# vb000/LookOnceToHear

Measured on AMD Instinct MI355X. Metric: frames_per_sec (5 s 16 kHz binaural clips, 625 STFT frames each, offline forward), higher is better.
Workload: dtype f32 via f16x3 split (3x fp16 MFMA per product, fp32 accumulate; ~22-bit operands, un-normalised rows scaled by a power of two before the split: any finite fp32 range); 1 GPU; BASELINE configs[2]: 32 x 5 s 16 kHz binaural clips per GPU, offline forward (configs/tsh.json separator, random-init weights); batch_per_gpu=32, global_batch=32, parallelism=utterance-dp1, gemm_mode=f16x3, tune=, batches_in_flight=1

## Files before the change

include/lookonce_hip.h:

```cpp
#ifndef LOOKONCE_HIP_H
#define LOOKONCE_HIP_H

#ifdef __cplusplus
extern "C" {
#endif

typedef void* lh_stream_t;

enum {
    LH_OK = 0,
    LH_ERR_ARG = 1,
    LH_ERR_UNSUPPORTED = 2,
    LH_ERR_LAUNCH = 3,
    LH_ERR_RANGE = 4
};

int lh_range_status(unsigned* range_flag, lh_stream_t stream);
int lh_range_flag_copy(unsigned* range_flag, void* host_pinned, lh_stream_t stream);
int lh_range_flag_clear(unsigned* range_flag, lh_stream_t stream);
int lh_selftest_fp16_subnormal(lh_stream_t stream);

enum { LH_GEMM_F32 = 0, LH_GEMM_F16X3 = 1 };

int lh_abi_version(void);
// ... 54 lines not shown
int lh_ring_advance_rows(int* pos, const int* write_pos, int modulo, int n_rows, lh_stream_t stream);

int lh_proj_ln_res(const float* merged, const void* w_pk, const float* bias, const float* slope,
                   const float* ln_w, const float* ln_b, const float* y2, const float* gain, float* out, int B,
                   int T, lh_stream_t stream);
int lh_proj_ln_res_fan(const float* merged, const void* w_pk, const float* bias, const float* slope, const float* ln_w,
                       const float* ln_b, const float* y2, const float* gain, float* out, int B, int T, int K,
                       lh_stream_t stream);
int lh_proj_ln_res_fan_win(const float* merged, const void* w_pk, const float* bias, const float* slope, const float* ln_w,
                           const float* ln_b, const float* y2, const float* gain, float* out, int B, int T, int t0, int Tc,
                           int K, lh_stream_t stream);

int lh_deconv_istft(const float* y, const float* deconv_buf_in, float* deconv_buf_out, const float* istft_buf_in,
                    float* istft_buf_out, const void* wdec_pk, const float* bdec, const void* wfb_dec,
                    float* wave_out, unsigned* range_flag, int keep_nonfinite, int B, int T, lh_stream_t stream);

int lh_intra_block_win(const float* x, const void* w_pk, const float* b_sum, const void* wlin_pk, const float* blin,
                       float* out, int B, int T, int t0, int Tc, lh_stream_t stream);
int lh_inter_block_win(const float* x, const void* w_pk, const float* b_sum, const void* wlin_pk, const float* blin,
                       const float* h0, const float* c0, float* hN, float* cN, float* out, int B, int T, int t0, int Tc,
                       int carry, lh_stream_t stream);
int lh_ln_lstm_intra_win(const float* x, const float* ln_w, const float* ln_b, const void* w_pk, const float* b_sum, float* h_out,
                         int B, int T, int t0, int Tc, lh_stream_t stream);
int lh_linear_res_win(const float* h, const void* w_pk, const float* bias, const float* res, float* out, int B, int T, int t0,
                      int Tc, int K, lh_stream_t stream);
int lh_inter_matvec_win(const float* x, const void* wih_pk, const float* b_sum, const float* whh, const void* wlin_pk,
                        const float* blin, const float* h0, const float* c0, float* hN, float* cN, float* out, int B, int T,
                        int t0, int Tc, int carry, lh_stream_t stream);
int lh_qkv_proj_ln_win(const float* y, const void* w_pk, const float* bias, const float* slopes, const float* lnq_w,
                       const float* lnq_b, const float* lnk_w, const float* lnk_b, const float* lnv_w,
// ... 153 lines not shown
```

lookoncetohear_amd/_cabi.py:

```python
from __future__ import annotations

import ctypes
import os
from ctypes import c_double, c_int, c_ulonglong, c_void_p

_PKG = os.path.dirname(os.path.abspath(__file__))
HIP_LIB_PATH = os.path.join(_PKG, "_lookonce_hip.so")
ABI_VERSION = 25

_P, _I = c_void_p, c_int
SIGNATURES = {
    "lh_abi_version": [],
    "lh_check_config": [_I] * 10,
    "lh_stft_conv_in": [_P] * 7 + [_I] * 3 + [_P],
    "lh_embed_proj_ln": [_P] * 7 + [_I, _P],
    "lh_set_tuning": [_I, _I],
    "lh_ln_lstm_intra": [_P] * 6 + [_I, _I, _P],
    "lh_ln_lstm_inter": [_P] * 10 + [_I, _I, _I, _P],
    "lh_intra_stream": [_P] * 5 + [_I, _P],
    "lh_inter_matvec": [_P] * 11 + [_I, _I, _P],
    "lh_intra_block": [_P] * 6 + [_I, _P],
    "lh_inter_block": [_P] * 10 + [_I, _I, _P],
    "lh_linear_res": [_P] * 5 + [_I, _I, _P],
    "lh_qkv_proj_ln": [_P] * 14 + [_I, _I, _P],
# ... 26 lines not shown
    "lh_resample": [_P, _P, _P] + [_I] * 6 + [_P],
    "lh_session_resample_in": [_P, _I, _P, _I, _P, _P, _I, _I, _P, _I, _I, _I, _P],
    "lh_session_resample_out": [_P, _P, _P, _P, _I, _I, _P, _I, _I, _I, _P],
    "lh_proj_ln_res": [_P] * 9 + [_I, _I, _P],
    "lh_deconv_istft": [_P] * 10 + [_I, _I, _I, _P],
    "lh_intra_block_win": [_P] * 6 + [_I, _I, _I, _I, _P],
    "lh_inter_block_win": [_P] * 10 + [_I, _I, _I, _I, _I, _P],
    "lh_ln_lstm_intra_win": [_P] * 6 + [_I, _I, _I, _I, _P],
    "lh_linear_res_win": [_P] * 5 + [_I, _I, _I, _I, _I, _P],
    "lh_inter_matvec_win": [_P] * 11 + [_I, _I, _I, _I, _I, _P],
    "lh_qkv_proj_ln_win": [_P] * 14 + [_I, _I, _I, _I, _P],
    "lh_local_attn_win": [_P] * 4 + [_I, _I, _I, _I, _P],
    "lh_proj_ln_res_win": [_P] * 9 + [_I, _I, _I, _I, _P],
    "lh_proj_ln_res_fan": [_P] * 9 + [_I, _I, _I, _P],
    "lh_proj_ln_res_fan_win": [_P] * 9 + [_I, _I, _I, _I, _I, _P],
    "lh_emb_frontend": [_P] * 10 + [_I, _I, _I, _P],
    "lh_emb_axis_fused": [_P] * 8 + [_I, _I, _I, _I, _I, _P],
    "lh_emb_axis_mv": [_P] * 9 + [_I, _I, _I, _I, _P],
    "lh_emb_attn_block": [_P] * 24 + [_I, _I, _P],
    "lh_emb_head": [_P] * 7 + [_I, _I, _P],
    "lh_render_binaural": [_P] * 8 + [_I, _I, _I, _I, _P],
    "lh_path_nearest": [_P] * 4 + [_I] * 5 + [_P],
    "lh_render_moving": [_P] * 10 + [_I] * 8 + [_P],
    "lh_metric_sums": [_P] * 8 + [_I, _I, _I, _P],
    "lh_binaural_cues": [_P] * 5 + [_I, _I, _I, _I, c_double, _P],
    "lh_range_status": [_P, _P],
    "lh_range_flag_copy": [_P, _P, _P],
    "lh_range_flag_clear": [_P, _P],
    "lh_selftest_fp16_subnormal": [_P],
    "lh_comm_unique_id": [_P],
# ... 119 lines not shown
```

lookoncetohear_amd/csrc/lh_backend.hip:

```cpp
#include "lh_split.h"

namespace lh {

constexpr int BE_NT = 512;
constexpr int BE_TT = 15;
constexpr int BE_NJ = BE_TT + 1;
constexpr int BE_NP = 36;
constexpr int BE_PP = 40;
constexpr int BE_SK = 7;
constexpr int BE_SA = BE_SK * 4 * BE_NJ * 8;
constexpr int BE_FP = NFFT + 4;
constexpr int BE_NLD = (NF * 16 + BE_NT - 1) / BE_NT;
#if !defined(BE_RING_N)
#define BE_RING_N 2
#endif
constexpr int BE_RING = BE_RING_N;
#if defined(LH_PROBE_TRACE)
__device__ unsigned long long lh_be_trace_buf[32];
#if defined(LH_PROBE_TRACE_T1)
#define BE_STAMP(k) do { if (blockIdx.x == 0 && tid == 0) lh_be_trace_buf[k] = __builtin_amdgcn_s_memtime(); } while (0)
#else
#define BE_STAMP(k) do { if (blockIdx.x == 3 && tid == 0 && tk == k0_ + 2) lh_be_trace_buf[k] = __builtin_amdgcn_s_memtime(); } while (0)
#endif
#else
// ... 336 lines not shown
            wave_out[((long)b * NSRC + s) * L + (long)(t0 + jt) * HOP + n] = (nf && !keep_nonfinite) ? 0.f : v;
            bad |= nf;
        }
        if (bad && range_flag) __hip_atomic_store(range_flag, 1u, __ATOMIC_RELAXED, __HIP_MEMORY_SCOPE_SYSTEM);
        __syncthreads();
        for (int i = tid; i < 2 * (FR_RP - NF) * 16; i += BE_NT) {
            const int img = i / ((FR_RP - NF) * 16), e = i % ((FR_RP - NF) * 16);
            *reinterpret_cast<f16x4*>(&ahi[img * FR_A + a_index<FR_RP>(NF + (e >> 4), (e & 15) * 4)]) = f16x4{0, 0, 0, 0};
        }
        BE_STAMP(10);
        }
        if (++tk == k1) run += gridDim.x;
    }
}

static int g_runs_per_b = 0;
int backend_set_runs(int v) {
    if (v < 0) return LH_ERR_ARG;
    g_runs_per_b = v;
    return LH_OK;
}

}

#if defined(LH_PROBE_TRACE)
extern "C" int lh_probe_be_trace_read(unsigned long long* host_dst) {
    return hipMemcpyFromSymbol(host_dst, HIP_SYMBOL(lh::lh_be_trace_buf), sizeof(lh::lh_be_trace_buf)) == hipSuccess ? 0 : 1;
}
#endif

// ... 4 lines not shown
    using namespace lh;
    if (!y || !deconv_buf_in || !deconv_buf_out || !istft_buf_in || !istft_buf_out || !wdec_pk || !bdec || !wfb_dec ||
        !wave_out || B <= 0 || T <= 0)
        return LH_ERR_ARG;
    if (deconv_buf_in == deconv_buf_out || istft_buf_in == istft_buf_out) return LH_ERR_ARG;
    const int tiles_per_b = (T + BE_TT - 1) / BE_TT;
    int runs_per_b = g_runs_per_b ? g_runs_per_b : 256 / B;
    runs_per_b = runs_per_b < 1 ? 1 : (runs_per_b > tiles_per_b ? tiles_per_b : runs_per_b);
    const int n_runs = B * runs_per_b;
    hipLaunchKernelGGL(k_deconv_istft, dim3(n_runs < 256 ? n_runs : 256), dim3(BE_NT), 0, (hipStream_t)stream, y,
                       deconv_buf_in, deconv_buf_out, istft_buf_in, istft_buf_out, (const _Float16*)wdec_pk, bdec,
                       (const _Float16*)wfb_dec, wave_out, range_flag, keep_nonfinite, B, T, runs_per_b);
    return check_launch();
}

namespace lh {
__global__ void k_range_fetch(unsigned* flag) { flag[1] = atomicExch(&flag[0], 0u); }
}
static int range_fetch(unsigned* flag, lh_stream_t stream) {
    if (!flag) return LH_ERR_ARG;
    hipLaunchKernelGGL(lh::k_range_fetch, dim3(1), dim3(1), 0, (hipStream_t)stream, flag);
    return lh::check_launch();
}
extern "C" int lh_range_flag_copy(unsigned* flag, void* host_pinned, lh_stream_t stream) {
    if (!host_pinned) return LH_ERR_ARG;
    const int rc = range_fetch(flag, stream);
    if (rc != LH_OK) return rc;
    return hipMemcpyAsync(host_pinned, flag + 1, sizeof(unsigned), hipMemcpyDeviceToHost, (hipStream_t)stream) == hipSuccess
               ? LH_OK : LH_ERR_LAUNCH;
}
// ... 40 lines not shown
```

lookoncetohear_amd/csrc/lh_frontend.hip:

```cpp
#include "lh_split.h"

namespace lh {

constexpr int FE_NTH = 512;
constexpr int FE_TT = 14;
constexpr int FE_NJ = 16;
constexpr int FE_AP = NFFT + 8;
constexpr int FE_SP = 68;
constexpr int FE_NT = (NK + 15) / 16;
constexpr int FE_KS = NFFT / 32;
constexpr int FE_OP = C + 4;

__global__ void __launch_bounds__(FE_NTH, 1) k_stft_conv_in(const float* __restrict__ x, const float* __restrict__ cbuf_in,
                                                            float* __restrict__ cbuf_out, const _Float16* __restrict__ wfb_pk,
                                                            const _Float16* __restrict__ wc_pk, const float* __restrict__ bc,
                                                            float* __restrict__ z, int B, int T, int n_samples) {
    __shared__ __attribute__((aligned(16))) _Float16 ahi[NMIC * FE_NJ * FE_AP];
    __shared__ __attribute__((aligned(16))) _Float16 alo[NMIC * FE_NJ * FE_AP];
    __shared__ __attribute__((aligned(16))) _Float16 sth[(NF + 2) * FE_SP];
    __shared__ __attribute__((aligned(16))) _Float16 stl[(NF + 2) * FE_SP];
    __shared__ __attribute__((aligned(16))) float outs[2][NF * FE_OP];
    __shared__ float tmax[FE_NTH / 64];
    const int tid = threadIdx.x, lane = tid & 63, wave = wave_id(tid), g4 = lane >> 4, l15 = lane & 15;

// ... 262 lines not shown
}

extern "C" int lh_embed_proj_ln_rows(const float* embed, const float* w, const float* bias, const float* ln_w,
                                     const float* ln_b, float* scratch, float* gain, const lh_snap_item_t* items, int n_items,
                                     int S, lh_stream_t stream) {
    using namespace lh;
    if (!embed || !w || !bias || !ln_w || !ln_b || !scratch || !gain || scratch == gain || !items || S <= 0 || n_items < 1 ||
        n_items > S)
        return LH_ERR_ARG;
    hipLaunchKernelGGL(k_embed_proj_rows, dim3((C * NF + EP_ROWS - 1) / EP_ROWS, (n_items + EP_NB - 1) / EP_NB), dim3(256), 0,
                       (hipStream_t)stream, embed, w, bias, scratch, items, n_items, S);
    hipLaunchKernelGGL(k_embed_ln_rows, dim3(n_items), dim3(256), 0, (hipStream_t)stream, scratch, ln_w, ln_b, gain, items, S);
    return check_launch();
}

extern "C" int lh_abi_version(void) { return 25; }

extern "C" int lh_check_config(int nfft, int hop, int n_mics, int emb_dim, int n_blocks_unused, int lstm_hidden,
                               int n_heads, int attn_window, int n_srcs, int spk_emb_dim) {
    using namespace lh;
    (void)n_blocks_unused;
    if (nfft != NFFT || hop != HOP || n_mics != NMIC || emb_dim != C || lstm_hidden != H || n_heads != NH ||
        attn_window != WIN || n_srcs != NSRC || spk_emb_dim != SPK)
        return LH_ERR_UNSUPPORTED;
    return LH_OK;
}
```

lookoncetohear_amd/csrc/lh_pointwise.hip:

```cpp
#include "lh_split.h"
#include <type_traits>

namespace lh {

template <int K>
__global__ void __launch_bounds__(256) k_linear_res(const float* __restrict__ h, const _Float16* __restrict__ w_pk,
                                                    const float* __restrict__ bias, const float* __restrict__ res,
                                                    float* __restrict__ out, int rows, int seg, long segstride) {
    auto grow = [&](long r) -> long { return (r / seg) * segstride + r % seg; };
    constexpr int KS = K / 32, RP = 64, CP = C + 4;
    __shared__ __attribute__((aligned(16))) _Float16 ahi[KS * 4 * RP * 8];
    __shared__ __attribute__((aligned(16))) _Float16 alo[KS * 4 * RP * 8];
    __shared__ __attribute__((aligned(16))) float cs[RP * CP];
    const int tid = threadIdx.x, lane = tid & 63, wave = wave_id(tid), g4 = lane >> 4, l15 = lane & 15;

    f16x8 wh[KS], wl[KS];
    load_w<KS>(w_pk, wave, lane, wh, wl);
    const float bz = bias[wave * 16 + l15];

    const int ntiles = (rows + RP - 1) / RP;
    for (int tile = blockIdx.x; tile < ntiles; tile += gridDim.x) {
        const long r0 = (long)tile * RP;
        constexpr int NLD = RP * (K / 4) / 256;
        float4 stg[NLD];
// ... 262 lines not shown
        QKV_STAMP(5);
    }
}
#if defined(LH_PROBE_TRACE)
}
extern "C" int lh_probe_qkv_trace_read(unsigned long long* host_dst) {
    return hipMemcpyFromSymbol(host_dst, HIP_SYMBOL(lh::lh_qkv_trace_buf), sizeof(lh::lh_qkv_trace_buf)) == hipSuccess ? 0 : 1;
}
namespace lh {
#endif

#if defined(LH_DBG_K6)
__device__ unsigned lh_dbg_k6[4];
__device__ float lh_dbg_part[8 * 24 * 256 * 4];
#endif
template <bool FAN>
__global__ void __launch_bounds__(256, 2) k_proj_ln_res(const float* __restrict__ merged, const _Float16* __restrict__ w_pk,
                                                     const float* __restrict__ bias, const float* __restrict__ slope,
                                                     const float* __restrict__ lnw, const float* __restrict__ lnb,
                                                     const float* __restrict__ y2, const float* __restrict__ gain,
                                                     float* __restrict__ out, int T, int nframes, int Tc, int tw0, int nfan) {
    constexpr int YP = C + 4;
    auto gidx = [&](int fr) -> long { return (long)(fr / Tc) * T + tw0 + fr % Tc; };
    __shared__ __attribute__((aligned(16))) _Float16 ahi[FR_A];
    __shared__ __attribute__((aligned(16))) _Float16 alo[FR_A];
    __shared__ __attribute__((aligned(16))) float ys[NF * YP];
    __shared__ float red[4];
    const int tid = threadIdx.x, lane = tid & 63, wave = wave_id(tid), g4 = lane >> 4, l15 = lane & 15;

    f16x8 wh[2], wl[2];
    load_w<2>(w_pk, wave, lane, wh, wl);
    const float bz = bias[wave * 16 + l15];
    const float a = slope[0];
    constexpr int N = NF * C, N4 = N / 4;
    constexpr int NSLOT = (N4 + 255) / 256;
    float4 pw[NSLOT], pb[NSLOT];
#pragma unroll
    for (int k = 0; k < NSLOT; ++k) {
        const int i = min(tid + 256 * k, N4 - 1);
        pw[k] = *reinterpret_cast<const float4*>(&lnw[i * 4]);
        pb[k] = *reinterpret_cast<const float4*>(&lnb[i * 4]);
    }

// ... 80 lines not shown
#pragma unroll
                for (int k = 0; k < NSLOT; ++k)
                    rv[k] = *reinterpret_cast<const float4*>(&gj[(long)min(tid + 256 * k, N4 - 1) * 4]);
#pragma unroll
                for (int k = 0; k < NSLOT; ++k) pin_here(rv[k]);
#pragma unroll
                for (int k = 0; k < NSLOT; ++k) {
                    rv[k].x = v[k].x * rv[k].x; rv[k].y = v[k].y * rv[k].y; rv[k].z = v[k].z * rv[k].z; rv[k].w = v[k].w * rv[k].w;
                }
#pragma unroll
                for (int k = 0; k < NSLOT; ++k) {
                    const int i = tid + 256 * k;
                    if (i < N4) *reinterpret_cast<float4*>(&out[fo + i * 4]) = rv[k];
                }
            }
            continue;
        }
        if (gain) {
#pragma unroll
            for (int k = 0; k < NSLOT; ++k)
                rv[k] = *reinterpret_cast<const float4*>(&gain[(long)b * N + (long)min(tid + 256 * k, N4 - 1) * 4]);
#pragma unroll
            for (int k = 0; k < NSLOT; ++k) {
                v[k].x *= rv[k].x; v[k].y *= rv[k].y; v[k].z *= rv[k].z; v[k].w *= rv[k].w;
            }
        }
#pragma unroll
        for (int k = 0; k < NSLOT; ++k) {
            const int i = tid + 256 * k;
            if (i < N4) *reinterpret_cast<float4*>(&out[fr + i * 4]) = v[k];
// ... 67 lines not shown
        return LH_ERR_ARG;
    hipLaunchKernelGGL(k_qkv_proj_ln<true>, dim3(B < 512 ? B : 512), dim3(256), 0, (hipStream_t)stream, y,
                       (const _Float16*)w_pk, bias, slopes, lnq_w, lnq_b, lnk_w, lnk_b, lnv_w, lnv_b, (_Float16*)q,
                       (_Float16*)kx, (_Float16*)vx, 1, B, write_pos, 1, 0);
    return check_launch();
}

extern "C" int lh_proj_ln_res_win(const float* merged, const void* w_pk, const float* bias, const float* slope,
                                  const float* ln_w, const float* ln_b, const float* y2, const float* gain, float* out,
                                  int B, int T, int t0, int Tc, lh_stream_t stream) {
    using namespace lh;
    if (!merged || !w_pk || !bias || !slope || !ln_w || !ln_b || !y2 || !out || B <= 0 || T <= 0 || t0 < 0 || Tc <= 0 ||
        t0 + Tc > T)
        return LH_ERR_ARG;
    const int nframes = B * Tc;
    hipLaunchKernelGGL(k_proj_ln_res<false>, dim3(nframes < 512 ? nframes : 512), dim3(256), 0, (hipStream_t)stream, merged,
                       (const _Float16*)w_pk, bias, slope, ln_w, ln_b, y2, gain, out, T, nframes, Tc, t0, 1);
    return check_launch();
}

extern "C" int lh_proj_ln_res(const float* merged, const void* w_pk, const float* bias, const float* slope,
                              const float* ln_w, const float* ln_b, const float* y2, const float* gain, float* out,
                              int B, int T, lh_stream_t stream) {
    return lh_proj_ln_res_win(merged, w_pk, bias, slope, ln_w, ln_b, y2, gain, out, B, T, 0, T, stream);
}

extern "C" int lh_proj_ln_res_fan_win(const float* merged, const void* w_pk, const float* bias, const float* slope,
                                      const float* ln_w, const float* ln_b, const float* y2, const float* gain, float* out,
                                      int B, int T, int t0, int Tc, int K, lh_stream_t stream) {
    using namespace lh;
    if (!gain || K < 1) return LH_ERR_ARG;
    if (K == 1) return lh_proj_ln_res_win(merged, w_pk, bias, slope, ln_w, ln_b, y2, gain, out, B, T, t0, Tc, stream);
    if (!merged || !w_pk || !bias || !slope || !ln_w || !ln_b || !y2 || !out || B <= 0 || T <= 0 || t0 < 0 || Tc <= 0 ||
        t0 + Tc > T)
        return LH_ERR_ARG;
    const int nframes = B * Tc;
    hipLaunchKernelGGL(k_proj_ln_res<true>, dim3(nframes < 512 ? nframes : 512), dim3(256), 0, (hipStream_t)stream, merged,
                       (const _Float16*)w_pk, bias, slope, ln_w, ln_b, y2, gain, out, T, nframes, Tc, t0, K);
    return check_launch();
}

extern "C" int lh_proj_ln_res_fan(const float* merged, const void* w_pk, const float* bias, const float* slope,
                                  const float* ln_w, const float* ln_b, const float* y2, const float* gain, float* out,
                                  int B, int T, int K, lh_stream_t stream) {
    return lh_proj_ln_res_fan_win(merged, w_pk, bias, slope, ln_w, ln_b, y2, gain, out, B, T, 0, T, K, stream);
}

#if defined(LH_DBG_K6)
extern "C" int lh_dbg_part_read(float* host) {
    return hipMemcpyFromSymbol(host, HIP_SYMBOL(lh::lh_dbg_part), sizeof(lh::lh_dbg_part)) == hipSuccess ? 0 : 1;
}
extern "C" int lh_dbg_k6_read(unsigned* host4, int reset) {
    if (hipMemcpyFromSymbol(host4, HIP_SYMBOL(lh::lh_dbg_k6), 16) != hipSuccess) return 1;
// ... 5 lines not shown
```

lookoncetohear_amd/net.py:

```python
from __future__ import annotations

import ctypes
import math
import os
from typing import Dict, Optional, Tuple

import numpy as np
import torch
import torch.nn as nn
import torch.nn.functional as F

from . import _cabi
from .weights import KV_PAD_ROWS, QK_PAD, pack_all, unsplit_qk, unsplit_v


def mod_pad(x: torch.Tensor, chunk_size: int, pad: Tuple[int, int]):
    mod = 0
    if x.shape[-1] % chunk_size != 0:
        mod = chunk_size - (x.shape[-1] % chunk_size)
    if mod or pad[0] or pad[1]:
        x = F.pad(x, (pad[0], mod + pad[1]))
    return x, mod


# ... 159 lines not shown
            raise NotImplementedError("only the chunk-causal attention mode of configs/tsh.json is implemented")
        shape = (self.nfft, stft_chunk_size, num_ch, D, H, L, local_atten_len, num_src, embed_dim)
        if shape != (192, 128, 2, 64, 64, 4, 50, 2, 256):
            raise NotImplementedError(
                f"the gfx950 kernels are specialised on the configs/tsh.json shapes; got (nfft, hop, mics, D, H, L, "
                f"window, srcs, embed_dim) = {shape}")
        self.E = math.ceil(512 * 1.0 / self.n_freqs)
        self.V_dim = D // L
        self.tfgridnet = _TFGridNetParams(self.nfft, stft_chunk_size, num_ch, num_src, D, B, H, L, embed_dim)
        self.gemm_mode = os.environ.get("LOOKONCE_GEMM", "f16x3")
        self._check_gemm_mode()
        rc = os.environ.get("LOOKONCE_RANGE_CHECK", "1")
        self.range_check = False if rc == "0" else ("sync" if rc == "sync" else True)
        self._range_flags: Dict[str, torch.Tensor] = {}
        self.fuse_linear = os.environ.get("LOOKONCE_FUSE", "1") != "0"
        self.fuse_intra_min_frames = int(os.environ.get("LOOKONCE_FUSE_INTRA_MIN_FRAMES", "6000"))
        self.inter_matvec_max_seqs = int(os.environ.get("LOOKONCE_MATVEC_MAX_SEQS", "256"))
        self.stream_intra_max_frames = 128
        self.n_cus = 256
        self.time_chunks = int(os.environ.get("LOOKONCE_TIME_CHUNKS", "0"))
        self.time_chunks_small = int(os.environ.get("LOOKONCE_TIME_CHUNKS_SMALL", "0"))
        self.chunk_min_frames = 64
        self._chunk_streams: Dict[str, list] = {}
        self._pack_key = None
        self._packed = None
        self._ws: Dict[tuple, dict] = {}
        self._zeros: Dict[tuple, dict] = {}
        self._blob = None
        self._debug_taps: Optional[dict] = None
        self._prof: Optional[list] = None
# ... 218 lines not shown
                    e1.record()
                    prof.append((name, e0, e1))

            lib_, lib = lib, _Timed

            conv_in = c32(state["conv_buf"]); conv_out = new(conv_in)
            lib.call("lh_stft_conv_in", P(x), P(conv_in), P(conv_out), P(pk["wfb_t"]), P(pk["conv_w"]),
                     P(pk["conv_b"]), P(xa), Bn, T, ns, st)
            lib.call("lh_embed_proj_ln", P(embed), P(pk["emb_w"]), P(pk["emb_b"]), P(pk["emb_ln_w"]),
                     P(pk["emb_ln_b"]), P(ws["gain_raw"]), P(ws["gain"]), Bn, st)
            if taps is not None:
                taps["Z0"], taps["G"] = xa.clone(), ws["gain"].clone()

            mode = 1 if self.gemm_mode == "f16x3" else 0
            K = self._n_time_chunks(Bn, T, mode)
            if K > 1:
                self._blocks_chunked(lib, pk, ws, state, Bn, T, dev, from_zero, want_state, K)
            else:
                self._blocks_whole(lib, pk, ws, state, Bn, T, dev, from_zero, want_state, mode)

            dec_in, ist_in = c32(state["deconv_buf"]), c32(state["istft_buf"])
            dec_out, ist_out = new(dec_in), new(ist_in)
            y = torch.empty(Bn, self.n_srcs, hop * T, device=dev, dtype=torch.float32)
            flag = self._range_flag(dev)
            lib.call("lh_deconv_istft", P(xa), P(dec_in), P(dec_out), P(ist_in), P(ist_out), P(pk["deconv_w"]),
                     P(pk["deconv_b"]), P(pk["wfb_dec"]), P(y), P(flag), 1, Bn, T, st)
            if want_state:
                state["conv_buf"], state["deconv_buf"], state["istft_buf"] = conv_out, dec_out, ist_out
            if self.range_check == "sync" and not self._capturing():
                if self.range_status(dev):
                    raise RuntimeError(self._RANGE_MSG.format("this forward"))
        return y, (state if want_state else None)

    def _separate_many(self, x: torch.Tensor, embeds: torch.Tensor) -> torch.Tensor:
        if self.training and torch.is_grad_enabled():
            raise RuntimeError("lookoncetohear_amd.Net is an inference-only drop-in (forward kernels, no autograd): call "
                               ".eval() and/or run under torch.no_grad(); training stays on the reference model")
        self._check_gemm_mode()
        assert x.shape[1] == self.num_ch, "input must be [B, num_ch, N]"
        Bn, _, n = x.shape
        Kt = embeds.shape[1]
        Bk = Bn * Kt
        embed = embeds.reshape(Bk, -1)
        if self.gemm_mode == "f32all" or self.n_blocks < 2:
            y, _ = self._separate(x.repeat_interleave(Kt, 0), embed, None, False)
            return y.view(Bn, Kt, *y.shape[1:])
        lib = self._lib(x)
# ... 27 lines not shown
                K = self._n_time_chunks(rows, T, mode)
                if K > 1:
                    self._blocks_chunked(lib, pk, w, s, rows, T, dev, True, False, K, blocks, f)
                else:
                    self._blocks_whole(lib, pk, w, s, rows, T, dev, True, False, mode, blocks, f)
            dec_in, ist_in = c32(sk["deconv_buf"]), c32(sk["istft_buf"])
            dec_out, ist_out = new(dec_in), new(ist_in)
            y = torch.empty(Bn, Kt, self.n_srcs, hop * T, device=dev, dtype=torch.float32)
            lib.call("lh_deconv_istft", P(wsk["xa"]), P(dec_in), P(dec_out), P(ist_in), P(ist_out), P(pk["deconv_w"]),
                     P(pk["deconv_b"]), P(pk["wfb_dec"]), P(y), P(self._range_flag(dev)), 1, Bk, T, st)
            if self.range_check == "sync" and not self._capturing():
                if self.range_status(dev):
                    raise RuntimeError(self._RANGE_MSG.format("this forward"))
        return y

    def _blocks_whole(self, lib, pk, ws, state, Bn, T, dev, from_zero, want_state, mode, blocks=None, fan=None):
        F_, nh, H_, hist = self.n_freqs, self.n_head, self.hidden, self.local_atten_len - 1
        P = lambda t: t.data_ptr()
        new = lambda t: torch.empty_like(t, dtype=torch.float32)
        c32 = lambda t: t.contiguous().float()
        xa, xb, xc, hbuf = ws["xa"], ws["xb"], ws["xc"], ws["hbuf"]
        st = self._stream(dev)
        taps = self._debug_taps
        rows = Bn * T * F_
        wkey, bkey = ("_w16", "_b16") if mode else ("_w", "_b")
        for i in (range(self.n_blocks) if blocks is None else blocks):
            bp = pk["blocks"][i]
            bs = state["gridnet_bufs"][f"buf{i}"]
            h0, c0 = c32(bs["h0"]), c32(bs["c0"])
            hN, cN = new(h0), new(c0)
            fuse = mode == 1 and self.fuse_linear
# ... 26 lines not shown
                ws["hist_dirty"] = True
            elif ws["hist_dirty"]:
                ws["kx"][:, :hist].zero_()
                ws["vx"][:, :hist].zero_()
                ws["hist_dirty"] = False
            lib.call("lh_qkv_proj_ln", P(xc), P(bp["qkv_w"]), P(bp["qkv_b"]), P(bp["qkv_slopes"]), P(bp["lnq_w"]),
                     P(bp["lnq_b"]), P(bp["lnk_w"]), P(bp["lnk_b"]), P(bp["lnv_w"]), P(bp["lnv_b"]), P(ws["q"]),
                     P(ws["kx"]), P(ws["vx"]), None, Bn, T, st)
            lib.call("lh_local_attn", P(ws["q"]), P(ws["kx"]), P(ws["vx"]), P(xb), Bn, T, st)
            if taps is not None:
                taps[f"blocks.{i}.attn"] = xb.clone()
            gain = ws["gain"] if (i == 0 and self.n_blocks > 1) else None
            if fan is not None and i == 0:
                lib.call("lh_proj_ln_res_fan", P(xb), P(bp["proj_w"]), P(bp["proj_b"]), P(bp["proj_slope"]),
                         P(bp["proj_ln_w"]), P(bp["proj_ln_b"]), P(xc), P(fan[0]), P(fan[1]), Bn, T, fan[2], st)
            else:
                lib.call("lh_proj_ln_res", P(xb), P(bp["proj_w"]), P(bp["proj_b"]), P(bp["proj_slope"]),
                         P(bp["proj_ln_w"]), P(bp["proj_ln_b"]), P(xc), P(gain) if gain is not None else None, P(xa),
                         Bn, T, st)
            if want_state:
                bs["h0"], bs["c0"] = hN, cN
                bs["K_buf"] = torch.empty(Bn * nh, hist, self.E * F_, device=dev, dtype=torch.float32)
                bs["V_buf"] = torch.empty(Bn * nh, hist, self.V_dim * F_, device=dev, dtype=torch.float32)
                lib.call("lh_ring_unpack", P(ws["kx"]), P(ws["vx"]), P(bs["K_buf"]), P(bs["V_buf"]), Bn, T, st)
            if taps is not None:
                taps[f"blocks.{i}.Y2"] = xc.clone()
                taps[f"blocks.{i}.Q"] = unsplit_qk(ws["q"], self.E * F_)
                taps[f"blocks.{i}.K"] = unsplit_qk(ws["kx"][:, hist:hist + T], self.E * F_)
                taps[f"blocks.{i}.V"] = unsplit_v(ws["vx"][:, hist:hist + T])
                taps[f"blocks.{i}.out"] = xa.clone()
# ... 28 lines not shown
        if Bn * self.n_freqs <= self.inter_matvec_max_seqs:
            align = 64
        cuts = [(k * T) // K for k in range(K + 1)]
        if T // K >= 2 * align or (align == 64 and T // K >= 64):
            cuts = [0] + [int(round(k * T / K / align)) * align for k in range(1, K)] + [T]
        return cuts

    def _lanes(self, dev, K) -> _Lanes:
        pool = self._chunk_streams.setdefault(str(dev), [])
        while len(pool) < K - 1:
            pool.append(torch.cuda.Stream(device=dev))
        if self.chunk_min_frames < self.local_atten_len - 1:
            raise ValueError("chunk_min_frames must cover the attention history (49 frames) on concurrent streams")
        return _Lanes(dev, pool[:K - 1])

    def _blocks_chunked(self, lib, pk, ws, state, Bn, T, dev, from_zero, want_state, K, blocks=None, fan=None):
        blocks = range(self.n_blocks) if blocks is None else blocks
        F_, nh, hist = self.n_freqs, self.n_head, self.local_atten_len - 1
        P = lambda t: t.data_ptr()
        c32 = lambda t: t.contiguous().float()
        xa, xb, xc = ws["xa"], ws["xb"], ws["xc"]
        lanes = self._lanes(dev, K)
        unfused_intra = Bn * T < self.fuse_intra_min_frames
        matvec_inter = Bn * F_ <= self.inter_matvec_max_seqs
        if "kxb" not in ws:
            z16 = lambda *s_: torch.zeros(*s_, device=dev, dtype=torch.float16)
            ws["kxb"] = [ws["kx"]] + [z16(*ws["kx"].shape) for _ in range(self.n_blocks - 1)]
            ws["vxb"] = [ws["vx"]] + [z16(*ws["vx"].shape) for _ in range(self.n_blocks - 1)]
            ws["hist_dirty_b"] = [False] * self.n_blocks
        bounds = self._window_bounds(Bn, T, K)
        hs, cs = {}, {}
# ... 45 lines not shown
                                 t0, Tc, carry, st)
                    if k + 1 < K:
                        ev_r = lanes.signal(k)
                    lib.call("lh_qkv_proj_ln_win", P(xc), P(bp["qkv_w"]), P(bp["qkv_b"]), P(bp["qkv_slopes"]), P(bp["lnq_w"]),
                             P(bp["lnq_b"]), P(bp["lnk_w"]), P(bp["lnk_b"]), P(bp["lnv_w"]), P(bp["lnv_b"]), P(ws["q"]),
                             P(kx), P(vx), None, Bn, T, t0, Tc, st)
                    ev_prev = ev_q
                    if k + 1 < K:
                        ev_q = lanes.signal(k)
                    if k > 0:
                        lanes.wait(k, ev_prev)
                    lib.call("lh_local_attn_win", P(ws["q"]), P(kx), P(vx), P(xb), Bn, T, t0, Tc, st)
                    if fan is not None and i == 0:
                        lib.call("lh_proj_ln_res_fan_win", P(xb), P(bp["proj_w"]), P(bp["proj_b"]), P(bp["proj_slope"]),
                                 P(bp["proj_ln_w"]), P(bp["proj_ln_b"]), P(xc), P(fan[0]), P(fan[1]), Bn, T, t0, Tc, fan[2], st)
                    else:
                        lib.call("lh_proj_ln_res_win", P(xb), P(bp["proj_w"]), P(bp["proj_b"]), P(bp["proj_slope"]),
                                 P(bp["proj_ln_w"]), P(bp["proj_ln_b"]), P(xc), P(gain) if gain is not None else None, P(xa),
                                 Bn, T, t0, Tc, st)
        lanes.join()
        if want_state:
            for i in blocks:
                bs = state["gridnet_bufs"][f"buf{i}"]
                bs["h0"], bs["c0"] = hs[i][K].reshape(1, -1, self.hidden), cs[i][K].reshape(1, -1, self.hidden)
                bs["K_buf"] = torch.empty(Bn * nh, hist, self.E * F_, device=dev, dtype=torch.float32)
                bs["V_buf"] = torch.empty(Bn * nh, hist, self.V_dim * F_, device=dev, dtype=torch.float32)
                lib.call("lh_ring_unpack", P(ws["kxb"][i]), P(ws["vxb"][i]), P(bs["K_buf"]), P(bs["V_buf"]), Bn, T,
                         self._stream(dev))

    def _check_gemm_mode(self):
# ... 1183 lines not shown
```

Baseline: 2.914 million frames/s.

## Fuse deconv tap products into last block's projection and simplify iSTFT kernel

The last block's proj+LN+residual kernel now also computes the 3x3 deconvolution tap products per frequency with MFMA and writes them out with a per-frame max. A new taps_istft kernel then only sums the taps over the time and frequency neighbours, splits the result and runs the synthesis GEMM. This removes the separate deconv GEMM pass over the full-width final features. The cost is an extra intermediate buffer (36 floats per frequency and frame), more shared memory in the projection kernel, and a conservative scaling bound based on the weight norms.

```diff
diff --git a/include/lookonce_hip.h b/include/lookonce_hip.h
--- a/include/lookonce_hip.h
+++ b/include/lookonce_hip.h
@@ -92,6 +92,15 @@
 int lh_deconv_istft(const float* y, const float* deconv_buf_in, float* deconv_buf_out, const float* istft_buf_in,
                     float* istft_buf_out, const void* wdec_pk, const float* bdec, const void* wfb_dec,
                     float* wave_out, unsigned* range_flag, int keep_nonfinite, int B, int T, lh_stream_t stream);
+
+int lh_proj_ln_res_taps(const float* merged, const void* w_pk, const float* bias, const float* slope, const float* ln_w,
+                        const float* ln_b, const float* y2, const void* wdec_pk, float* p_out, float* fmax, int B, int T,
+                        lh_stream_t stream);
+int lh_proj_ln_res_taps_win(const float* merged, const void* w_pk, const float* bias, const float* slope, const float* ln_w,
+                            const float* ln_b, const float* y2, const void* wdec_pk, float* p_out, float* fmax, int B, int T,
+                            int t0, int Tc, lh_stream_t stream);
+int lh_taps_istft(const float* p, const float* fmax, const void* wdec_pk, const float* bdec, const void* wfb_dec,
+                  float* wave_out, unsigned* range_flag, int keep_nonfinite, int B, int T, lh_stream_t stream);
 
 int lh_intra_block_win(const float* x, const void* w_pk, const float* b_sum, const void* wlin_pk, const float* blin,
                        float* out, int B, int T, int t0, int Tc, lh_stream_t stream);
diff --git a/lookoncetohear_amd/_cabi.py b/lookoncetohear_amd/_cabi.py
--- a/lookoncetohear_amd/_cabi.py
+++ b/lookoncetohear_amd/_cabi.py
@@ -6,7 +6,7 @@
 
 _PKG = os.path.dirname(os.path.abspath(__file__))
 HIP_LIB_PATH = os.path.join(_PKG, "_lookonce_hip.so")
-ABI_VERSION = 25
+ABI_VERSION = 26
 
 _P, _I = c_void_p, c_int
 SIGNATURES = {
@@ -64,6 +64,9 @@
     "lh_proj_ln_res_win": [_P] * 9 + [_I, _I, _I, _I, _P],
     "lh_proj_ln_res_fan": [_P] * 9 + [_I, _I, _I, _P],
     "lh_proj_ln_res_fan_win": [_P] * 9 + [_I, _I, _I, _I, _I, _P],
+    "lh_proj_ln_res_taps": [_P] * 10 + [_I, _I, _P],
+    "lh_proj_ln_res_taps_win": [_P] * 10 + [_I, _I, _I, _I, _P],
+    "lh_taps_istft": [_P] * 7 + [_I, _I, _I, _P],
     "lh_emb_frontend": [_P] * 10 + [_I, _I, _I, _P],
     "lh_emb_axis_fused": [_P] * 8 + [_I, _I, _I, _I, _I, _P],
     "lh_emb_axis_mv": [_P] * 9 + [_I, _I, _I, _I, _P],
diff --git a/lookoncetohear_amd/csrc/lh_backend.hip b/lookoncetohear_amd/csrc/lh_backend.hip
--- a/lookoncetohear_amd/csrc/lh_backend.hip
+++ b/lookoncetohear_amd/csrc/lh_backend.hip
@@ -374,6 +374,197 @@
     }
 }
 
+constexpr int TI_PQ = NF * BE_NP / 4;
+constexpr int TI_NLD = (TI_PQ + BE_NT - 1) / BE_NT;
+constexpr int TI_RING = 4;
+
+__global__ void __launch_bounds__(BE_NT) k_taps_istft(const float* __restrict__ p, const float* __restrict__ fmax,
+                                                      const _Float16* __restrict__ wd_pk, const float* __restrict__ bd,
+                                                      const _Float16* __restrict__ wfb_pk, float* __restrict__ wave_out,
+                                                      unsigned* __restrict__ range_flag, int keep_nonfinite, int B, int T,
+                                                      int runs_per_b) {
+    __shared__ __attribute__((aligned(16))) float pring[4][NF + 2][BE_PP];
+    __shared__ __attribute__((aligned(16))) _Float16 sxh[NSRC * BE_SA];
+    __shared__ __attribute__((aligned(16))) _Float16 sxl[NSRC * BE_SA];
+    __shared__ __attribute__((aligned(16))) float frs[BE_NJ][NSRC][BE_FP];
+    __shared__ float fmaxr[4];
+    __shared__ __attribute__((aligned(16))) float sinv[BE_NJ];
+    __shared__ float w1s[48];
+    const int tid = threadIdx.x, lane = tid & 63, wave = wave_id(tid), g4 = lane >> 4, l15 = lane & 15;
+
+    const bool synth = wave < 6;
+    float bias4[4];
+#pragma unroll
+    for (int o = 0; o < 4; ++o) bias4[o] = bd[o];
+    const float bmax = fmaxf(fmaxf(fabsf(bias4[0]), fabsf(bias4[1])), fmaxf(fabsf(bias4[2]), fabsf(bias4[3])));
+    if (tid < 4) fmaxr[tid] = 0.f;
+    if (tid < BE_NJ) sinv[tid] = 0.f;
+    if (tid < 48) {
+        float a = 0.f;
+        for (int k = 0; k < C; ++k) {
+            const int idx = (((tid >> 4) * 2 + (k >> 5)) * 64 + ((k >> 3) & 3) * 16 + (tid & 15)) * 16 + (k & 7);
+            a += fabsf((float)wd_pk[idx]) + fabsf((float)wd_pk[idx + 8]);
+        }
+        w1s[tid] = a;
+    }
+    static_assert((NSRC * BE_SA) % 8 == 0, "16-byte zero fill");
+    const f16x8 z8 = f16x8{0, 0, 0, 0, 0, 0, 0, 0};
+    for (int i = tid; i < NSRC * BE_SA / 8; i += BE_NT) {
+        *reinterpret_cast<f16x8*>(&sxh[i * 8]) = z8;
+        *reinterpret_cast<f16x8*>(&sxl[i * 8]) = z8;
+    }
+    for (int i = tid; i < 4 * (NF + 2) * BE_PP; i += BE_NT) (&pring[0][0][0])[i] = 0.f;
+    __syncthreads();
+    float W1 = 0.f;
+    for (int i = 0; i < 48; ++i) W1 = fmaxf(W1, w1s[i]);
+    W1 *= 3.0f;
+
+    const int tiles_per_b = (T + BE_TT - 1) / BE_TT;
+    const int n_runs = B * runs_per_b;
+    const long L = (long)HOP * T;
+    int run = blockIdx.x, tk = 0, k1 = 0;
+    for (;;) {
+        bool first = false;
+        if (tk == k1) {
+            if (run >= n_runs) break;
+            const int rb0 = run % runs_per_b;
+            tk = (int)((long)tiles_per_b * rb0 / runs_per_b);
+            k1 = (int)((long)tiles_per_b * (rb0 + 1) / runs_per_b);
+            first = true;
+        }
+        const int b = run / runs_per_b;
+        {
+        const int t0 = tk * BE_TT;
+        const int nt_out = min(BE_TT, T - t0);
+        const bool cont = !first;
+        const int tv = tid + (tk >> 30);
+        __syncthreads();
+
+        auto put_sx = [&](int jd, int s, int k, float v) {
+            _Float16 h, l;
+            split_hl(v, h, l);
+            const int idx = s * BE_SA + a_index<BE_NJ>(jd, k);
+            sxh[idx] = h;
+            sxl[idx] = l;
+        };
+        if (t0 == 0) {
+            static_assert(NSRC * NK <= BE_NT, "one carried spectrum value per thread");
+            float sc, iv;
+            pow2_scale<12>(0.f, sc, iv);
+            if (tid < NSRC * NK) put_sx(0, tid / NK, tid % NK, 0.f * sc);
+            if (tid == 0) sinv[0] = iv;
+        } else if (cont) {
+            for (int i = tid; i < NSRC * NK; i += BE_NT) {
+                const int s = i / NK, k = i % NK;
+                const int src = s * BE_SA + a_index<BE_NJ>(BE_TT, k), dst = s * BE_SA + a_index<BE_NJ>(0, k);
+                sxh[dst] = sxh[src];
+                sxl[dst] = sxl[src];
+            }
+            if (tid == 0) sinv[0] = sinv[BE_TT];
+        }
+
+        struct PFrame { f32x4 a, b; float m; };
+        static_assert(TI_NLD == 2 && TI_RING == 4, "two float4 per thread and frame, two pairs of frames in flight");
+        PFrame r0, r1, r2, r3;
+        const unsigned eoff0 = (unsigned)tv * 16u, eoff1 = (unsigned)min(tv + BE_NT, TI_PQ - 1) * 16u;
+        const char* pb = reinterpret_cast<const char*>(p) + (long)b * T * (TI_PQ * 16);
+        const float* fb = fmax + (long)b * T;
+        auto load_frame_p = [&](int fr, PFrame& d) __attribute__((always_inline)) {
+            const char* base = pb + (long)fr * (TI_PQ * 16);
+            d.a = *reinterpret_cast<const f32x4*>(base + eoff0);
+            d.b = *reinterpret_cast<const f32x4*>(base + eoff1);
+            d.m = fb[fr];
+        };
+        static_assert(BE_NP == 36, "9 float4 per row of P");
+        auto put_frame = [&](int slot, const PFrame& s) __attribute__((always_inline)) {
+            *reinterpret_cast<f32x4*>(&pring[slot][tv / 9 + 1][(tv % 9) * 4]) = s.a;
+            const int j = tv + BE_NT;
+            if (j < TI_PQ) *reinterpret_cast<f32x4*>(&pring[slot][j / 9 + 1][(j % 9) * 4]) = s.b;
+        };
+        const int fr_first = cont ? t0 : max(t0 - 3, -2);
+        const int fr_end = t0 + nt_out;
+        auto pair = [&](int fr, PFrame& x, PFrame& y) __attribute__((always_inline)) {
+            const bool two = fr + 1 < fr_end;
+            __syncthreads();
+            if (fr < 0) {
+                for (int i = tv; i < 2 * NF * BE_PP; i += BE_NT) pring[2 + i / (NF * BE_PP)][1 + (i / BE_PP) % NF][i % BE_PP] = 0.f;
+                if (tid < 2) fmaxr[2 + tid] = 0.f;
+            } else {
+                put_frame((fr + 4) & 3, x);
+                if (two) put_frame((fr + 5) & 3, y);
+                if (tid == 0) {
+                    fmaxr[(fr + 4) & 3] = x.m;
+                    if (two) fmaxr[(fr + 5) & 3] = y.m;
+                }
+            }
+            load_frame_p(min(fr + TI_RING, fr_end - 1), x);
+            load_frame_p(min(fr + 1 + TI_RING, fr_end - 1), y);
+            __syncthreads();
+
+            for (int i = tv; i < (two ? 2 : 1) * NF; i += BE_NT) {
+                const int q = i >= NF, f = i - NF * q;
+                const int td = fr + q;
+                if (td < t0 - 1 || td < 0) continue;
+                const int jd = td + 1 - t0;
+                float4 v = make_float4(bias4[0], bias4[1], bias4[2], bias4[3]);
+#pragma unroll
+                for (int kt = 0; kt < 3; ++kt) {
+                    const int ps = (td - kt + 4) & 3;
+#pragma unroll
+                    for (int kf = 0; kf < 3; ++kf) {
+                        const float4 pv = *reinterpret_cast<const float4*>(&pring[ps][f + 2 - kf][(kt * 3 + kf) * 4]);
+                        v.x += pv.x; v.y += pv.y; v.z += pv.z; v.w += pv.w;
+                    }
+                }
+                const float vo[4] = {v.x, v.y, v.z, v.w};
+                float ssx, isx;
+                pow2_scale<14>(fmaf(W1, fmaxr[(td + 4) & 3] + fmaxr[(td + 3) & 3] + fmaxr[(td + 2) & 3], bmax), ssx, isx);
+                if (f == 0) sinv[jd] = isx;
+#pragma unroll
+                for (int o = 0; o < 4; ++o) put_sx(jd, o >> 1, (o & 1) * NF + f, vo[o] * ssx);
+            }
+        };
+        if (fr_first >= 0) { load_frame_p(min(fr_first, fr_end - 1), r0); load_frame_p(min(fr_first + 1, fr_end - 1), r1); }
+        load_frame_p(min(fr_first + 2, fr_end - 1), r2);
+        load_frame_p(min(fr_first + 3, fr_end - 1), r3);
+        for (int fbase = fr_first; fbase < fr_end; fbase += TI_RING) {
+            pair(fbase, r0, r1);
+            if (fbase + 2 < fr_end) pair(fbase + 2, r2, r3);
+        }
+        __syncthreads();
+
+        if (synth) {
+#pragma unroll 1
+            for (int i = 0; i < 2; ++i) {
+                f16x8 wfh[BE_SK], wfl[BE_SK];
+                load_w<BE_SK>(wfb_pk, 2 * wave + i, lane, wfh, wfl);
+#pragma unroll
+                for (int s = 0; s < NSRC; ++s) {
+                    const f32x4 acc = mma_tile<BE_NJ, BE_SK>(sxh + s * BE_SA, sxl + s * BE_SA, 0, g4, l15, wfh, wfl, 0.f);
+                    const float4 iv4 = *reinterpret_cast<const float4*>(&sinv[g4 * 4]);
+                    const float iv[4] = {iv4.x, iv4.y, iv4.z, iv4.w};
+#pragma unroll
+                    for (int r = 0; r < 4; ++r) frs[g4 * 4 + r][s][(2 * wave + i) * 16 + l15] = acc[r] * iv[r];
+                }
+            }
+        }
+        __syncthreads();
+
+        bool bad = false;
+        for (int i = tid; i < nt_out * NSRC * HOP; i += BE_NT) {
+            const int n = i % HOP, s = (i / HOP) % NSRC, jt = i / (HOP * NSRC);
+            float v = frs[jt + 1][s][n];
+            if (n < NFFT - HOP) v += frs[jt][s][n + HOP];
+            const bool nf = (__float_as_uint(v) & 0x7f800000u) == 0x7f800000u;
+            wave_out[((long)b * NSRC + s) * L + (long)(t0 + jt) * HOP + n] = (nf && !keep_nonfinite) ? 0.f : v;
+            bad |= nf;
+        }
+        if (bad && range_flag) __hip_atomic_store(range_flag, 1u, __ATOMIC_RELAXED, __HIP_MEMORY_SCOPE_SYSTEM);
+        }
+        if (++tk == k1) run += gridDim.x;
+    }
+}
+
 static int g_runs_per_b = 0;
 int backend_set_runs(int v) {
     if (v < 0) return LH_ERR_ARG;
@@ -408,6 +599,20 @@
     return check_launch();
 }
 
+extern "C" int lh_taps_istft(const float* p, const float* fmax, const void* wdec_pk, const float* bdec, const void* wfb_dec,
+                             float* wave_out, unsigned* range_flag, int keep_nonfinite, int B, int T, lh_stream_t stream) {
+    using namespace lh;
+    if (!p || !fmax || !wdec_pk || !bdec || !wfb_dec || !wave_out || B <= 0 || T <= 0) return LH_ERR_ARG;
+    const int tiles_per_b = (T + BE_TT - 1) / BE_TT;
+    int runs_per_b = g_runs_per_b ? g_runs_per_b : 256 / B;
+    runs_per_b = runs_per_b < 1 ? 1 : (runs_per_b > tiles_per_b ? tiles_per_b : runs_per_b);
+    const int n_runs = B * runs_per_b;
+    hipLaunchKernelGGL(k_taps_istft, dim3(n_runs < 256 ? n_runs : 256), dim3(BE_NT), 0, (hipStream_t)stream, p, fmax,
+                       (const _Float16*)wdec_pk, bdec, (const _Float16*)wfb_dec, wave_out, range_flag, keep_nonfinite, B, T,
+                       runs_per_b);
+    return check_launch();
+}
+
 namespace lh {
 __global__ void k_range_fetch(unsigned* flag) { flag[1] = atomicExch(&flag[0], 0u); }
 }
diff --git a/lookoncetohear_amd/csrc/lh_frontend.hip b/lookoncetohear_amd/csrc/lh_frontend.hip
--- a/lookoncetohear_amd/csrc/lh_frontend.hip
+++ b/lookoncetohear_amd/csrc/lh_frontend.hip
@@ -300,7 +300,7 @@
     return check_launch();
 }
 
-extern "C" int lh_abi_version(void) { return 25; }
+extern "C" int lh_abi_version(void) { return 26; }
 
 extern "C" int lh_check_config(int nfft, int hop, int n_mics, int emb_dim, int n_blocks_unused, int lstm_hidden,
                                int n_heads, int attn_window, int n_srcs, int spk_emb_dim) {
diff --git a/lookoncetohear_amd/csrc/lh_pointwise.hip b/lookoncetohear_amd/csrc/lh_pointwise.hip
--- a/lookoncetohear_amd/csrc/lh_pointwise.hip
+++ b/lookoncetohear_amd/csrc/lh_pointwise.hip
@@ -300,19 +300,31 @@
 __device__ unsigned lh_dbg_k6[4];
 __device__ float lh_dbg_part[8 * 24 * 256 * 4];
 #endif
-template <bool FAN>
+constexpr int TAP_NP = 36;
+constexpr int TAP_W = 3 * 2 * 64 * 16;
+template <bool FAN, bool TAPS = false>
 __global__ void __launch_bounds__(256, 2) k_proj_ln_res(const float* __restrict__ merged, const _Float16* __restrict__ w_pk,
                                                      const float* __restrict__ bias, const float* __restrict__ slope,
                                                      const float* __restrict__ lnw, const float* __restrict__ lnb,
                                                      const float* __restrict__ y2, const float* __restrict__ gain,
-                                                     float* __restrict__ out, int T, int nframes, int Tc, int tw0, int nfan) {
+                                                     float* __restrict__ out, int T, int nframes, int Tc, int tw0, int nfan,
+                                                     const _Float16* __restrict__ wd_pk, float* __restrict__ fmax) {
+    static_assert(!(FAN && TAPS), "the tap products are the last block's output: no gain, no fan-out");
     constexpr int YP = C + 4;
     auto gidx = [&](int fr) -> long { return (long)(fr / Tc) * T + tw0 + fr % Tc; };
     __shared__ __attribute__((aligned(16))) _Float16 ahi[FR_A];
     __shared__ __attribute__((aligned(16))) _Float16 alo[FR_A];
     __shared__ __attribute__((aligned(16))) float ys[NF * YP];
     __shared__ float red[4];
+    __shared__ __attribute__((aligned(16))) _Float16 wds[TAPS ? TAP_W : 8];
+    __shared__ __attribute__((aligned(16))) float rinv[TAPS ? FR_RP : 4];
+    __shared__ float wm[4];
     const int tid = threadIdx.x, lane = tid & 63, wave = wave_id(tid), g4 = lane >> 4, l15 = lane & 15;
+    if (TAPS) {
+        for (int i = tid; i < TAP_W / 8; i += 256)
+            *reinterpret_cast<f16x8*>(&wds[i * 8]) = *reinterpret_cast<const f16x8*>(&wd_pk[i * 8]);
+        if (tid < FR_RP - NF) rinv[NF + tid] = 0.f;
+    }
 
     f16x8 wh[2], wl[2];
     load_w<2>(w_pk, wave, lane, wh, wl);
@@ -423,6 +435,73 @@
                     if (i < N4) *reinterpret_cast<float4*>(&out[fo + i * 4]) = rv[k];
                 }
             }
+            continue;
+        }
+        if (TAPS) {
+            const int tx = tid + (fidx >> 30);
+            float me = 0.f, mo = 0.f;
+#pragma unroll
+            for (int k = 0; k < NSLOT; k += 2) me = fmaxf(me, absmax4(v[k]));
+#pragma unroll
+            for (int k = 1; k < NSLOT; k += 2) mo = fmaxf(mo, absmax4(v[k]));
+            static_assert(NSLOT == 7 && N4 - 1 - 256 * (NSLOT - 1) == 15, "slot 6: row 96 in threads 0..15, the clamped last float4 elsewhere");
+            if (tid >= 16) mo = fmaxf(mo, absmax4(v[NSLOT - 1]));
+            const float ge = wave_max_uniform(me), go = wave_max_uniform(mo);
+            float sce, ive, sco, ivo;
+            pow2_scale<FR_TE>(ge, sce, ive);
+            pow2_scale<FR_TE>(go, sco, ivo);
+#pragma unroll
+            for (int k = 0; k < NSLOT; ++k) {
+                const int i = tx + 256 * k;
+                const float sc = (k & 1) ? sco : sce;
+                if (i < N4) {
+                    store_split4<FR_RP>(ahi, alo, i >> 4, (i & 15) * 4, make_float4(v[k].x * sc, v[k].y * sc, v[k].z * sc, v[k].w * sc));
+                    if ((i & 15) == 0) rinv[i >> 4] = (k & 1) ? ivo : ive;
+                }
+            }
+            if (lane == 0) wm[wave] = fmaxf(ge, go);
+            __syncthreads();
+#pragma unroll 1
+            for (int mt = wave; mt < FR_RP / 16; mt += 4) {
+                const int ln = lane + (mt >> 30);
+                f16x8 ah[2], al[2];
+#pragma unroll
+                for (int ks = 0; ks < 2; ++ks) {
+                    const int idx = a_slot<FR_RP>(ks * 4 + g4, mt * 16 + l15);
+                    ah[ks] = *reinterpret_cast<const f16x8*>(&ahi[idx]);
+                    al[ks] = *reinterpret_cast<const f16x8*>(&alo[idx]);
+                }
+                const float4 iv4 = *reinterpret_cast<const float4*>(&rinv[mt * 16 + g4 * 4]);
+                const float iv[4] = {iv4.x, iv4.y, iv4.z, iv4.w};
+#pragma unroll
+                for (int nt = 0; nt < 3; ++nt) {
+                    f32x4 am = f32x4{0.f, 0.f, 0.f, 0.f}, ac = f32x4{0.f, 0.f, 0.f, 0.f};
+#pragma unroll
+                    for (int ks = 0; ks < 2; ++ks) {
+                        const f16x8 th = *reinterpret_cast<const f16x8*>(&wds[((nt * 2 + ks) * 64 + ln) * 16]);
+                        const f16x8 tl = *reinterpret_cast<const f16x8*>(&wds[((nt * 2 + ks) * 64 + ln) * 16 + 8]);
+                        am = __builtin_amdgcn_mfma_f32_16x16x32_f16(ah[ks], th, am, 0, 0, 0);
+                        ac = __builtin_amdgcn_mfma_f32_16x16x32_f16(ah[ks], tl, ac, 0, 0, 0);
+                        ac = __builtin_amdgcn_mfma_f32_16x16x32_f16(al[ks], th, ac, 0, 0, 0);
+                    }
+                    const int col = nt * 16 + l15;
+#pragma unroll
+                    for (int r = 0; r < 4; ++r) {
+                        const int f = mt * 16 + g4 * 4 + r;
+                        if (f < NF && col < TAP_NP) ys[f * TAP_NP + col] = (am[r] + ac[r]) * iv[r];
+                    }
+                }
+            }
+            __syncthreads();
+            const long gf = gidx(fidx);
+            float* pd = out + gf * (NF * TAP_NP);
+            constexpr int PQ = NF * TAP_NP / 4;
+#pragma unroll
+            for (int k = 0; k < (PQ + 255) / 256; ++k) {
+                const int i = tx + 256 * k;
+                if (i < PQ) *reinterpret_cast<float4*>(&pd[i * 4]) = *reinterpret_cast<const float4*>(&ys[i * 4]);
+            }
+            if (tid == 0) fmax[gf] = fmaxf(fmaxf(wm[0], wm[1]), fmaxf(wm[2], wm[3]));
             continue;
         }
         if (gain) {
@@ -520,8 +599,9 @@
         t0 + Tc > T)
         return LH_ERR_ARG;
     const int nframes = B * Tc;
-    hipLaunchKernelGGL(k_proj_ln_res<false>, dim3(nframes < 512 ? nframes : 512), dim3(256), 0, (hipStream_t)stream, merged,
-                       (const _Float16*)w_pk, bias, slope, ln_w, ln_b, y2, gain, out, T, nframes, Tc, t0, 1);
+    hipLaunchKernelGGL((k_proj_ln_res<false, false>), dim3(nframes < 512 ? nframes : 512), dim3(256), 0, (hipStream_t)stream, merged,
+                       (const _Float16*)w_pk, bias, slope, ln_w, ln_b, y2, gain, out, T, nframes, Tc, t0, 1, (const _Float16*)nullptr,
+                       (float*)nullptr);
     return check_launch();
 }
 
@@ -529,6 +609,26 @@
                               const float* ln_w, const float* ln_b, const float* y2, const float* gain, float* out,
                               int B, int T, lh_stream_t stream) {
     return lh_proj_ln_res_win(merged, w_pk, bias, slope, ln_w, ln_b, y2, gain, out, B, T, 0, T, stream);
+}
+
+extern "C" int lh_proj_ln_res_taps_win(const float* merged, const void* w_pk, const float* bias, const float* slope,
+                                       const float* ln_w, const float* ln_b, const float* y2, const void* wdec_pk, float* p_out,
+                                       float* fmax, int B, int T, int t0, int Tc, lh_stream_t stream) {
+    using namespace lh;
+    if (!merged || !w_pk || !bias || !slope || !ln_w || !ln_b || !y2 || !wdec_pk || !p_out || !fmax || B <= 0 || T <= 0 ||
+        t0 < 0 || Tc <= 0 || t0 + Tc > T)
+        return LH_ERR_ARG;
+    const int nframes = B * Tc;
+    hipLaunchKernelGGL((k_proj_ln_res<false, true>), dim3(nframes < 512 ? nframes : 512), dim3(256), 0, (hipStream_t)stream,
+                       merged, (const _Float16*)w_pk, bias, slope, ln_w, ln_b, y2, (const float*)nullptr, p_out, T, nframes, Tc,
+                       t0, 1, (const _Float16*)wdec_pk, fmax);
+    return check_launch();
+}
+
+extern "C" int lh_proj_ln_res_taps(const float* merged, const void* w_pk, const float* bias, const float* slope,
+                                   const float* ln_w, const float* ln_b, const float* y2, const void* wdec_pk, float* p_out,
+                                   float* fmax, int B, int T, lh_stream_t stream) {
+    return lh_proj_ln_res_taps_win(merged, w_pk, bias, slope, ln_w, ln_b, y2, wdec_pk, p_out, fmax, B, T, 0, T, stream);
 }
 
 extern "C" int lh_proj_ln_res_fan_win(const float* merged, const void* w_pk, const float* bias, const float* slope,
@@ -541,8 +641,9 @@
         t0 + Tc > T)
         return LH_ERR_ARG;
     const int nframes = B * Tc;
-    hipLaunchKernelGGL(k_proj_ln_res<true>, dim3(nframes < 512 ? nframes : 512), dim3(256), 0, (hipStream_t)stream, merged,
-                       (const _Float16*)w_pk, bias, slope, ln_w, ln_b, y2, gain, out, T, nframes, Tc, t0, K);
+    hipLaunchKernelGGL((k_proj_ln_res<true, false>), dim3(nframes < 512 ? nframes : 512), dim3(256), 0, (hipStream_t)stream, merged,
+                       (const _Float16*)w_pk, bias, slope, ln_w, ln_b, y2, gain, out, T, nframes, Tc, t0, K, (const _Float16*)nullptr,
+                       (float*)nullptr);
     return check_launch();
 }
 
diff --git a/lookoncetohear_amd/net.py b/lookoncetohear_amd/net.py
--- a/lookoncetohear_amd/net.py
+++ b/lookoncetohear_amd/net.py
@@ -197,6 +197,7 @@
         self.range_check = False if rc == "0" else ("sync" if rc == "sync" else True)
         self._range_flags: Dict[str, torch.Tensor] = {}
         self.fuse_linear = os.environ.get("LOOKONCE_FUSE", "1") != "0"
+        self.fuse_taps = os.environ.get("LOOKONCE_FUSE_TAPS", "1") != "0"
         self.fuse_intra_min_frames = int(os.environ.get("LOOKONCE_FUSE_INTRA_MIN_FRAMES", "6000"))
         self.inter_matvec_max_seqs = int(os.environ.get("LOOKONCE_MATVEC_MAX_SEQS", "256"))
         self.stream_intra_max_frames = 128
@@ -445,23 +446,40 @@
 
             mode = 1 if self.gemm_mode == "f16x3" else 0
             K = self._n_time_chunks(Bn, T, mode)
+            ptaps = None
+            if self.fuse_taps and from_zero and taps is None:
+                ptaps = self._tap_buffers(ws, Bn, T, dev, own=K > 1)
             if K > 1:
-                self._blocks_chunked(lib, pk, ws, state, Bn, T, dev, from_zero, want_state, K)
+                self._blocks_chunked(lib, pk, ws, state, Bn, T, dev, from_zero, want_state, K, ptaps=ptaps)
             else:
-                self._blocks_whole(lib, pk, ws, state, Bn, T, dev, from_zero, want_state, mode)
-
-            dec_in, ist_in = c32(state["deconv_buf"]), c32(state["istft_buf"])
-            dec_out, ist_out = new(dec_in), new(ist_in)
+                self._blocks_whole(lib, pk, ws, state, Bn, T, dev, from_zero, want_state, mode, ptaps=ptaps)
+
             y = torch.empty(Bn, self.n_srcs, hop * T, device=dev, dtype=torch.float32)
             flag = self._range_flag(dev)
-            lib.call("lh_deconv_istft", P(xa), P(dec_in), P(dec_out), P(ist_in), P(ist_out), P(pk["deconv_w"]),
-                     P(pk["deconv_b"]), P(pk["wfb_dec"]), P(y), P(flag), 1, Bn, T, st)
+            if ptaps is not None:
+                lib.call("lh_taps_istft", P(ptaps[0]), P(ptaps[1]), P(pk["deconv_w"]), P(pk["deconv_b"]), P(pk["wfb_dec"]),
+                         P(y), P(flag), 1, Bn, T, st)
+            else:
+                dec_in, ist_in = c32(state["deconv_buf"]), c32(state["istft_buf"])
+                dec_out, ist_out = new(dec_in), new(ist_in)
+                lib.call("lh_deconv_istft", P(xa), P(dec_in), P(dec_out), P(ist_in), P(ist_out), P(pk["deconv_w"]),
+                         P(pk["deconv_b"]), P(pk["wfb_dec"]), P(y), P(flag), 1, Bn, T, st)
             if want_state:
                 state["conv_buf"], state["deconv_buf"], state["istft_buf"] = conv_out, dec_out, ist_out
             if self.range_check == "sync" and not self._capturing():
                 if self.range_status(dev):
                     raise RuntimeError(self._RANGE_MSG.format("this forward"))
         return y, (state if want_state else None)
+
+    def _tap_buffers(self, ws, Bn, T, dev, own):
+        n = Bn * T * self.n_freqs * 36
+        if "fmax" not in ws:
+            ws["fmax"] = torch.empty(Bn * T, device=dev, dtype=torch.float32)
+        if not own:
+            return ws["xa"].view(-1)[:n], ws["fmax"]
+        if "ptaps" not in ws:
+            ws["ptaps"] = torch.empty(n, device=dev, dtype=torch.float32)
+        return ws["ptaps"], ws["fmax"]
 
     def _separate_many(self, x: torch.Tensor, embeds: torch.Tensor) -> torch.Tensor:
         if self.training and torch.is_grad_enabled():
@@ -519,7 +537,7 @@
                     raise RuntimeError(self._RANGE_MSG.format("this forward"))
         return y
 
-    def _blocks_whole(self, lib, pk, ws, state, Bn, T, dev, from_zero, want_state, mode, blocks=None, fan=None):
+    def _blocks_whole(self, lib, pk, ws, state, Bn, T, dev, from_zero, want_state, mode, blocks=None, fan=None, ptaps=None):
         F_, nh, H_, hist = self.n_freqs, self.n_head, self.hidden, self.local_atten_len - 1
         P = lambda t: t.data_ptr()
         new = lambda t: torch.empty_like(t, dtype=torch.float32)
@@ -576,6 +594,9 @@
             if fan is not None and i == 0:
                 lib.call("lh_proj_ln_res_fan", P(xb), P(bp["proj_w"]), P(bp["proj_b"]), P(bp["proj_slope"]),
                          P(bp["proj_ln_w"]), P(bp["proj_ln_b"]), P(xc), P(fan[0]), P(fan[1]), Bn, T, fan[2], st)
+            elif ptaps is not None and i == self.n_blocks - 1 and gain is None:
+                lib.call("lh_proj_ln_res_taps", P(xb), P(bp["proj_w"]), P(bp["proj_b"]), P(bp["proj_slope"]),
+                         P(bp["proj_ln_w"]), P(bp["proj_ln_b"]), P(xc), P(pk["deconv_w"]), P(ptaps[0]), P(ptaps[1]), Bn, T, st)
             else:
                 lib.call("lh_proj_ln_res", P(xb), P(bp["proj_w"]), P(bp["proj_b"]), P(bp["proj_slope"]),
                          P(bp["proj_ln_w"]), P(bp["proj_ln_b"]), P(xc), P(gain) if gain is not None else None, P(xa),
@@ -634,7 +655,7 @@
             raise ValueError("chunk_min_frames must cover the attention history (49 frames) on concurrent streams")
         return _Lanes(dev, pool[:K - 1])
 
-    def _blocks_chunked(self, lib, pk, ws, state, Bn, T, dev, from_zero, want_state, K, blocks=None, fan=None):
+    def _blocks_chunked(self, lib, pk, ws, state, Bn, T, dev, from_zero, want_state, K, blocks=None, fan=None, ptaps=None):
         blocks = range(self.n_blocks) if blocks is None else blocks
         F_, nh, hist = self.n_freqs, self.n_head, self.local_atten_len - 1
         P = lambda t: t.data_ptr()
@@ -710,6 +731,10 @@
                     if fan is not None and i == 0:
                         lib.call("lh_proj_ln_res_fan_win", P(xb), P(bp["proj_w"]), P(bp["proj_b"]), P(bp["proj_slope"]),
                                  P(bp["proj_ln_w"]), P(bp["proj_ln_b"]), P(xc), P(fan[0]), P(fan[1]), Bn, T, t0, Tc, fan[2], st)
+                    elif ptaps is not None and i == self.n_blocks - 1 and gain is None:
+                        lib.call("lh_proj_ln_res_taps_win", P(xb), P(bp["proj_w"]), P(bp["proj_b"]), P(bp["proj_slope"]),
+                                 P(bp["proj_ln_w"]), P(bp["proj_ln_b"]), P(xc), P(pk["deconv_w"]), P(ptaps[0]), P(ptaps[1]), Bn, T,
+                                 t0, Tc, st)
                     else:
                         lib.call("lh_proj_ln_res_win", P(xb), P(bp["proj_w"]), P(bp["proj_b"]), P(bp["proj_slope"]),
                                  P(bp["proj_ln_w"]), P(bp["proj_ln_b"]), P(xc), P(gain) if gain is not None else None, P(xa),
```

Measured after the change: 2.959 million frames/s (median of 6 runs). 1.02x the previous value.
